# Roy-Kid/ADMP

Hardware: AMD Instinct MI355X
Metric: ns/day (electrostatics get_forces per 1 fs step, polarizable PME incl. SCF, moving atoms) (higher is better)
Workload: dtype f64; 1 GPU; water_pol_1024 (BASELINE configs[1]): 1024 polarizable MPID waters = 3072 atoms, seeded liquid box L=31.289 A, rc 4 A, f64; n_atoms=3072, n_pairs=42510, pair_list=fixed during the timed steps, parallelism=single GPU

## Files before the change

admp_amd/_lib.py:

```python
import ctypes

import numpy as np
import os

_HERE = os.path.dirname(os.path.abspath(__file__))
LIB_PATH = os.environ.get('ADMP_HIP_LIB') or os.path.join(_HERE, 'lib', 'libadmp_hip.so')

_c = ctypes
_vp, _i32, _i64, _dbl = _c.c_void_p, _c.c_int, _c.c_int64, _c.c_double
_u32, _u64 = _c.c_uint32, _c.c_uint64
_dp = _c.POINTER(_c.c_double)
_ip = _c.POINTER(_c.c_int)

PROTOTYPES = {
    'admp_version': (_c.c_char_p, []),
    'admp_create': (_i32, [_c.POINTER(_vp), _i32, _i32]),
    'admp_destroy': (_i32, [_vp]),
    'admp_last_error': (_c.c_char_p, [_vp]),
    'admp_set_stream': (_i32, [_vp, _vp]),
    'admp_use_default_stream': (_i32, [_vp]),
    'admp_synchronize': (_i32, [_vp]),
    'admp_set_topology': (_i32, [_vp, _i32, _vp, _vp, _vp, _vp, _vp]),
    'admp_set_ewald': (_i32, [_vp, _dbl, _i32, _i32, _i32, _i32, _i32]),
    'admp_set_pairs': (_i32, [_vp, _i64, _vp, _i32]),
# ... 28 lines not shown
    'admp_md_virial': (_i32, [_vp, _i32, _vp, _vp, _vp, _vp, _u64, _u64, _vp]),
    'admp_md_scale': (_i32, [_vp, _i32, _vp, _vp, _dbl]),
    'admp_md_mts_plan': (_i32, [_vp, _i32, _i32, _vp, _vp, _i32, _vp, _vp, _i32]),
    'admp_md_mts_step': (_i32, [_vp, _i32, _vp, _vp, _vp, _vp, _dp, _dbl, _dbl, _i32, _dbl, _dbl, _u64, _u64, _vp, _vp]),
    'admp_md_mts_info': (_i32, [_vp, _c.POINTER(_i64)]),
    'admp_md_con_plan': (_i32, [_vp, _i32, _i32, _vp, _vp, _i32]),
    'admp_md_con_step': (_i32, [_vp, _i32, _vp, _vp, _vp, _vp, _dp, _dbl, _dbl, _dbl, _dbl, _u64, _u64, _dbl, _i32, _vp]),
    'admp_md_con_kick': (_i32, [_vp, _i32, _vp, _vp, _vp, _vp, _dp, _dbl, _dbl, _dbl, _i32, _vp, _vp]),
    'admp_md_con_project': (_i32, [_vp, _i32, _vp, _vp, _vp, _dp, _dbl, _i32, _vp]),
    'admp_md_con_info': (_i32, [_vp, _c.POINTER(_i64)]),
    'admp_md_mol_plan': (_i32, [_vp, _i32, _vp, _i32]),
    'admp_md_mol_sums': (_i32, [_vp, _i32, _vp, _vp, _vp, _vp, _dp, _u64, _u64, _vp]),
    'admp_md_mol_scale': (_i32, [_vp, _i32, _vp, _vp, _vp, _dp, _dbl, _dbl]),
    'admp_md_mol_info': (_i32, [_vp, _c.POINTER(_i64)]),
    'admp_md_fire_step': (_i32, [_vp, _i32, _vp, _vp, _vp, _vp, _dp, _dbl, _u64, _vp]),
    'admp_neighbor_count': (_i32, [_vp, _i32, _vp, _dp, _dbl, _c.POINTER(_i64)]),
    'admp_neighbor_fill': (_i32, [_vp, _vp]),
    'admp_set_pairs_from_positions': (_i32, [_vp, _vp, _dp, _dbl]),
    'admp_slab_configure': (_i32, [_vp, _i32, _i32]),
    'admp_slab_info': (_i32, [_vp, _c.POINTER(_i64)]),
    'admp_scf_stats': (_i32, [_vp, _c.POINTER(_i64), _i32]),
    'admp_xpass_stats': (_i32, [_vp, _c.POINTER(_i64), _i32]),
    'admp_plane_mfma_stats': (_i32, [_vp, _c.POINTER(_i64), _i32]),
    'admp_mesh_convolve': (_i32, [_vp, _dp, _i32, _vp, _i32, _dp, _ip]),
    'admp_pair_real': (_i32, [_vp, _vp, _dp, _vp, _vp, _vp, _i32, _dp, _dp, _vp, _vp, _i32, _i32, _i32, _dp, _vp, _vp, _vp, _ip]),
    'admp_pair_rider_stats': (_i32, [_vp, _c.POINTER(_i64), _i32]),
    'admp_mesh_spread': (_i32, [_vp, _vp, _dp, _vp, _vp, _vp, _vp, _i32, _i32, _i32, _vp, _ip]),
    'admp_mesh_gather': (_i32, [_vp, _vp, _dp, _vp, _vp, _vp, _vp, _vp, _i32, _i32, _dp, _vp, _vp, _vp, _ip]),
    'admp_set_comm': (_i32, [_vp, _vp]),
    'admp_slab_home': (_i32, [_vp, _vp, _ip, _ip]),
    'admp_rccl_unique_id': (_i32, [_vp]),
    'admp_rccl_create': (_i32, [_c.POINTER(_vp), _i32, _vp, _i32, _i32]),
    'admp_rccl_destroy': (_i32, [_vp]),
    'admp_rccl_abort': (_i32, [_vp]),
    'admp_rccl_stats': (_i32, [_vp, _c.POINTER(_i64), _c.POINTER(_i64), _i32]),
    'admp_rccl_all_reduce': (_i32, [_vp, _vp, _i64, _i32, _i32, _vp]),
    'admp_rccl_all_to_all_v': (_i32, [_vp, _vp, _c.POINTER(_i64), _vp, _c.POINTER(_i64), _i32, _vp]),
    'admp_rccl_shift': (_i32, [_vp, _vp, _vp, _i64, _i32, _i32, _vp]),
    'admp_rccl_version': (_i32, [_ip]),
    'admp_rccl_last_error': (_c.c_char_p, []),
    'admp_set_comm_rccl': (_i32, [_vp, _vp]),
    'admp_profile_enable': (_i32, [_vp, _i32]),
    'admp_profile_filter': (_i32, [_vp, _c.c_char_p]),
    'admp_profile_reset': (_i32, [_vp]),
    'admp_profile_count': (_i32, [_vp]),
    'admp_profile_entry': (_i32, [_vp, _i32, _c.POINTER(_c.c_char_p), _dp, _c.POINTER(_i64)]),
# ... 59 lines not shown
```

admp_amd/csrc/dft_kernels.hip:

```cpp
#include "dft_lines.h"
#include "env.h"
#include "mfma.h"
#include "plane_mfma_plan.h"

namespace admp {

int dft_tile_cols(int N) { return dft_cols(N, dft_kq(), 0, 0); }
template <class T, int KQ, int JS>
__global__ __launch_bounds__(kDftBlock) void k_dft_z_r2c(int N, int nlines, int NL, int TK, const T* __restrict__ mesh,
                                                        Cx<T>* __restrict__ spec, const Cx<T>* __restrict__ twg,
                                                        long mesh_stride, long spec_stride) {
  mesh += blockIdx.y * mesh_stride;
  spec += blockIdx.y * spec_stride;
  const int H = (N - 1) / 2, Kh = N / 2 + 1;
  Cx<T>* tw = reinterpret_cast<Cx<T>*>(dft_smem);
  Cx<T>* p = tw + N;
  T* x0 = reinterpret_cast<T*>(p + H * NL);
  T* xn = x0 + NL;
  const int line0 = blockIdx.x * NL;
  const int nl = min(NL, nlines - line0);
  for (int t = threadIdx.x; t < N; t += kDftBlock) tw[t] = twg[t];
  for (int t = threadIdx.x; t < H * nl; t += kDftBlock) {
    const int l = t / H, jj = t - l * H;
    const T* x = mesh + (long)(line0 + l) * N;
// ... 422 lines not shown
        const int jb = wrap_add(ebase[2 * e], b, N2), bz = ebase[2 * e + 1];
#pragma unroll
        for (int c = 0; c < 6; ++c) {
          const T v = P0 * w[24 + c] + P1 * w[30 + c] + P2 * w[36 + c];
          const int jc = wrap_add(bz, c, N3);
          T* dst;
          if (jc == 0) dst = &x0[jb];
          else if (jc <= H3) dst = &p[(jc - 1) * N2 + jb].re;
          else if (2 * jc == N3) dst = &xn[jb];
          else dst = &p[(N3 - 1 - jc) * N2 + jb].im;
          atomicAdd(dst, v);
        }
      }
      __syncthreads();
    }
  }
  for (int t = threadIdx.x; t < H3 * N2; t += kZyBlock) {
    const Cx<T> ab = p[t];
    p[t] = Cx<T>{ab.re + ab.im, ab.re - ab.im};
  }
}

template <class T, int SIGN>
__device__ __forceinline__ void dft_y_unit(const PlaneMfmaPlan& mp, int u, const Cx<T>* Z, const Cx<T>* tw, Cx<T>* out, int os) {
  typedef typename Mfma<T>::Acc Acc;
  const int N = mp.N, H = mp.H, mt = u % mp.MT, ct = u / mp.MT;
  const int lane = threadIdx.x & 63, hi = plane_mfma_pos0(lane);
  const int i = plane_mfma_tw_row(mt, lane), c = plane_mfma_col(ct, lane), comp = plane_mfma_comp(lane);
  TwIdx ti(i < H ? i : 0, hi, N);
  const bool live = c < mp.ncols;
  const T* zc = reinterpret_cast<const T*>(Z + (live ? c : 0)) + comp;
  const int rs = 2 * mp.ncols;
  struct Ops { Cx<T> w; T b[2]; };
  auto fetch = [&](Ops& o, int kk) {
    o.w = tw[ti.m];
    ti.step();
    const bool ok = live && kk < H;
    o.b[0] = ok ? zc[(1 + kk) * rs] : T(0);
    o.b[1] = ok ? zc[(N - 1 - kk) * rs] : T(0);
  };
  Acc P = {0, 0, 0, 0}, R = {0, 0, 0, 0};
  T s0 = T(0);
  auto mul = [&](const Ops& o) {
    s0 += o.b[0];
    P = Mfma<T>::mma(o.w.re, o.b[0], P);
    R = Mfma<T>::mma(o.w.im, o.b[1], R);
  };
  Ops A, B;
  fetch(A, hi);
  for (int kk = hi; kk < mp.KP; kk += 8) {
    const bool two = kk + 4 < mp.KP;
    if (two) fetch(B, kk + 4);
    mul(A);
    if (kk + 8 < mp.KP) fetch(A, kk + 8);
    if (two) mul(B);
  }
  const T x0 = zc[0], xn = (N & 1) ? T(0) : zc[(N / 2) * rs];
  T* o = reinterpret_cast<T*>(out + (live ? c : 0)) + comp;
#pragma unroll
  for (int r = 0; r < 4; ++r) {
    const int k = plane_mfma_out_k(mt, lane, r);
    const T other = __shfl_xor(R[r], 8, 64);
    if (live && k <= H) {
      T base = x0 + P[r];
      if ((N & 1) == 0) base += (k & 1) ? -xn : xn;
      const T q = comp ? T(SIGN) * other : -T(SIGN) * other;
      o[2 * (long)k * os] = base + q;
      o[2 * (long)(N - k) * os] = base - q;
    }
  }
  if (mt == 0) {
    T s1 = (hi & 1) ? s0 : -s0;
    s0 += __shfl_xor(s0, 16, 64); s1 += __shfl_xor(s1, 16, 64);
    s0 += __shfl_xor(s0, 32, 64); s1 += __shfl_xor(s1, 32, 64);
    if (hi == 0 && live) {
      o[0] = x0 + s0 + xn;
      if ((N & 1) == 0) o[2 * (long)(N / 2) * os] = x0 + s1 + (((N / 2) & 1) ? -xn : xn);
    }
  }
}

template <class T>
__device__ __forceinline__ void dft_z_unit(const PlaneMfmaZPlan& zp, int u, const Cx<T>* p, const T* x0, const T* xn,
                                           const Cx<T>* tw, Cx<T>* Z) {
  typedef typename Mfma<T>::Acc Acc;
  const int N = zp.N, H = zp.H, mt = u % zp.MT, lt = u / zp.MT;
  const int lane = threadIdx.x & 63, hi = lane >> 4;
  const int kt = plane_mfma_z_tw_k(zp, mt, lane), l = plane_mfma_z_line(lt, lane);
  TwIdx ti((kt <= N / 2 ? kt : 0) - 1, hi, N);
  const bool live = l < zp.nlines;
  const Cx<T>* pl = p + (live ? l : 0);
  struct Ops { Cx<T> w, v; };
  auto fetch = [&](Ops& o, int kk) {
    o.w = tw[ti.m];
    ti.step();
    o.v = (live && kk < H) ? pl[kk * zp.nlines] : Cx<T>{T(0), T(0)};
  };
  Acc P = {0, 0, 0, 0}, R = {0, 0, 0, 0};
  auto mul = [&](const Ops& o) {
    P = Mfma<T>::mma(o.w.re, o.v.re, P);
    R = Mfma<T>::mma(o.w.im, o.v.im, R);
  };
// ... 108 lines not shown
    }
    ZY_TRACE_END(4);
    return;
  }
  for (int task = threadIdx.x; task < TK2 * Kl; task += kZyBlock) {
    const int g = task / Kl, c = task - g * Kl;
    int k[KQ];
#pragma unroll
    for (int q = 0; q < KQ; ++q) k[q] = (g + q * TK2 < Kh2) ? g + q * TK2 : 0;
    Cx<T> Xk[KQ], Xnk[KQ];
    dft_pair_outputs_rows<T, -1, KQ>(N2, k, Kl, Z + c, tw2, Xk, Xnk);
#pragma unroll
    for (int q = 0; q < KQ; ++q) {
      const int kq = g + q * TK2;
      if (kq < Kh2) {
        out[(long)kq * Kh + kz0 + c] = Xk[q];
        if (kq != 0 && 2 * kq != N2) out[(long)(N2 - kq) * Kh + kz0 + c] = Xnk[q];
      }
    }
  }
  ZY_TRACE_END(4);
}

template <class T, int KQ>
__global__ __launch_bounds__(kZyBlock) void k_dft_yz_inv(int N2, int N3, const Cx<T>* __restrict__ spec, T* __restrict__ mesh,
                                                         const Cx<T>* __restrict__ tw2g, const Cx<T>* __restrict__ tw3g,
                                                         long mesh_stride, long spec_stride, T* __restrict__ accum) {
  __shared__ int s_lines[2 * 160 + 2];
  __shared__ int s_nlines;
  const ZyLayout<T> L(N2, N3);
  const int Kh = N3 / 2 + 1, H2 = (N2 - 1) / 2;
  Cx<T>* tw3 = reinterpret_cast<Cx<T>*>(dft_smem + L.tw3);
  Cx<T>* tw2 = reinterpret_cast<Cx<T>*>(dft_smem + L.tw2);
  Cx<T>* V = reinterpret_cast<Cx<T>*>(dft_smem + L.a);
  Cx<T>* Z = reinterpret_cast<Cx<T>*>(dft_smem + L.b);
  const Cx<T>* in = spec + blockIdx.y * spec_stride + (long)blockIdx.x * N2 * Kh;
  T* plane = mesh + blockIdx.y * mesh_stride + (long)blockIdx.x * N2 * N3;
  T* acc = accum ? accum + (long)blockIdx.x * N2 * N3 : nullptr;
  const int Kh2 = N2 / 2 + 1, TK2 = (Kh2 + KQ - 1) / KQ;
  const int g0 = (int)(((long)TK2 * blockIdx.z) / gridDim.z), g1 = (int)(((long)TK2 * (blockIdx.z + 1)) / gridDim.z);
  ZY_TRACE(0);
  for (int t = threadIdx.x; t < N3; t += kZyBlock) tw3[t] = tw3g[t];
  for (int t = threadIdx.x; t < N2; t += kZyBlock) tw2[t] = tw2g[t];
  if (threadIdx.x == 0) {
    int n = 0;
    for (int g = g0; g < g1; ++g)
      for (int q = 0; q < KQ; ++q) {
        const int kq = g + q * TK2;
        if (kq >= Kh2) continue;
        s_lines[n++] = kq;
        if (kq != 0 && 2 * kq != N2) s_lines[n++] = N2 - kq;
      }
    s_nlines = n;
  }
  for (int t = threadIdx.x; t < (H2 + 1) * Kh; t += kZyBlock) {
    const int jj = t / Kh, c = t - jj * Kh;
    if (jj == H2) {
      Z[c] = in[c];
      if ((N2 & 1) == 0) Z[(N2 / 2) * Kh + c] = in[(long)(N2 / 2) * Kh + c];
      continue;
    }
    const Cx<T> a = in[(long)(1 + jj) * Kh + c], b = in[(long)(N2 - 1 - jj) * Kh + c];
    Z[(1 + jj) * Kh + c] = Cx<T>{a.re + b.re, a.im + b.im};
    Z[(N2 - 1 - jj) * Kh + c] = Cx<T>{a.re - b.re, a.im - b.im};
  }
  __syncthreads();
  ZY_TRACE(1);
  for (int task = threadIdx.x; task < (g1 - g0) * Kh; task += kZyBlock) {
    const int g = g0 + task / Kh, c = task % Kh;
    int k[KQ];
#pragma unroll
    for (int q = 0; q < KQ; ++q) k[q] = (g + q * TK2 < Kh2) ? g + q * TK2 : 0;
    Cx<T> Xk[KQ], Xnk[KQ];
    dft_pair_outputs_rows<T, +1, KQ>(N2, k, Kh, Z + c, tw2, Xk, Xnk);
#pragma unroll
    for (int q = 0; q < KQ; ++q) {
      const int kq = g + q * TK2;
      if (kq < Kh2) {
        V[kq * Kh + c] = Xk[q];
        if (kq != 0 && 2 * kq != N2) V[(N2 - kq) * Kh + c] = Xnk[q];
      }
    }
  }
  __syncthreads();
  ZY_TRACE(2);
  const int TK3 = (Kh + KQ - 1) / KQ, nl = s_nlines;
  for (int task = threadIdx.x; task < nl * TK3; task += kZyBlock) {
    const int l = s_lines[task / TK3], g = task % TK3;
    int j[KQ];
#pragma unroll
    for (int q = 0; q < KQ; ++q) j[q] = (g + q * TK3 < Kh) ? g + q * TK3 : 0;
    const Cx<T>* v = V + l * Kh;
    T xj[KQ], xnj[KQ];
    irdft_pair_outputs<T, KQ>(N3, j, 1, v + 1, v[0].re, (N3 & 1) ? T(0) : v[N3 / 2].re, tw3, xj, xnj);
    T* x = plane + (long)l * N3;
    T* ac = acc ? acc + (long)l * N3 : nullptr;
#pragma unroll
    for (int q = 0; q < KQ; ++q) {
      const int jq = g + q * TK3;
      if (jq < Kh) {
        x[jq] = xj[q];
        if (ac) ac[jq] += xj[q];
        if (jq != 0 && 2 * jq != N3) {
          x[N3 - jq] = xnj[q];
          if (ac) ac[N3 - jq] += xnj[q];
        }
      }
    }
  }
  ZY_TRACE_END(3);
// ... 64 lines not shown
  const size_t sh = dft_x_fixed_bytes(N, sizeof(T), false) + dft_x_col_bytes(N, sizeof(T), false) * (size_t)NC;
  const dim3 grid((Kh + NCt - 1) / NCt, K[1], 1);
#define XMIX(NTP)                                                                                                          \
  k_dft_x_mix<T, 2, 1, NTP><<<grid, kDftBlock, sh, st>>>(N, Kh, NC, TK, (long)K[1] * Kh, (long)Kh, K[2],                    \
                                                         reinterpret_cast<Cx<T>*>(spec), tabs, mix,                        \
                                                         reinterpret_cast<const Cx<T>*>(tw), energies, slot, spec_stride / 2)
  if (ntp == 1) XMIX(1); else if (ntp == 2) XMIX(2); else XMIX(4);
#undef XMIX
}
template <class T>
bool dft_zy_fits(const int K[3]) {
  static const bool off = !env_flag("ADMP_DFT_PLANES", true);
  return !off && 2 * K[0] <= 256 && ZyLayout<T>(K[1], K[2]).total + 2048 <= 160 * 1024;
}
template <class T>
bool dft_zy_spread_fits(const int K[3], int na) {
  static const int mx = env_int("ADMP_FUSE_SPREAD_MAX", 8192);
  return sizeof(T) == 8 && na > 0 && na <= mx && na <= kZySpreadMaxAtoms && dft_zy_fits<T>(K) && zy_spread_sub<T>(K[1], K[2]) >= 16;
}
template <class T>
bool launch_dft_zy(hipStream_t st, const int K[3], const T* tw, T* mesh, T* spec, int inverse, int nb, long mesh_stride,
                   long spec_stride, T* accum, const PlaneSpread<T>* sp, int* mfma_share) {
  const size_t sh = ZyLayout<T>(K[1], K[2]).total;
  const bool mf = sizeof(T) == 8 && !inverse && env_flag("ADMP_DFT_PLANE_MFMA", true) &&
                  (plane_mfma_y_plan(K[1], (K[2] / 2 + 1) / 2, kZyBlock / 64).CT > 0 ||
                   plane_mfma_z_plan(K[2], 0, (K[2] / 2 + 1) / 2, K[1], kZyBlock / 64).MT > 0);
  if (mfma_share) *mfma_share = mf ? 1 : 0;
  const Cx<T>* t1 = reinterpret_cast<const Cx<T>*>(tw) + K[0];
  const Cx<T>* t2 = t1 + K[1];
  const dim3 grid(K[0], nb, 2);
  static size_t attr_set[2] = {0, 0};
  if (inverse) {
    auto kern = k_dft_yz_inv<T, 2>;
    if (attr_set[1] < sh) { (void)hipFuncSetAttribute((const void*)kern, hipFuncAttributeMaxDynamicSharedMemorySize, (int)sh); attr_set[1] = sh; }
    kern<<<grid, kZyBlock, sh, st>>>(K[1], K[2], reinterpret_cast<const Cx<T>*>(spec), mesh, t1, t2, mesh_stride, spec_stride / 2,
                                     nb == 1 ? accum : nullptr);
    return accum != nullptr && nb == 1;
  }
  if constexpr (sizeof(T) == 8) {
    if (mf) {
      static size_t attr_mf[2] = {0, 0};
      auto kern = sp ? k_dft_zy_fwd<T, 2, true, true> : k_dft_zy_fwd<T, 2, false, true>;
      size_t& have = attr_mf[sp ? 1 : 0];
      if (have < sh) { (void)hipFuncSetAttribute((const void*)kern, hipFuncAttributeMaxDynamicSharedMemorySize, (int)sh); have = sh; }
      kern<<<grid, kZyBlock, sh, st>>>(K[1], K[2], mesh, reinterpret_cast<Cx<T>*>(spec), t1, t2, mesh_stride, spec_stride / 2,
                                       sp ? *sp : PlaneSpread<T>());
      return false;
    }
  }
  if (sp) {
    static size_t attr_sp = 0;
    auto kern = k_dft_zy_fwd<T, 2, true>;
    if (attr_sp < sh) { (void)hipFuncSetAttribute((const void*)kern, hipFuncAttributeMaxDynamicSharedMemorySize, (int)sh); attr_sp = sh; }
    kern<<<grid, kZyBlock, sh, st>>>(K[1], K[2], mesh, reinterpret_cast<Cx<T>*>(spec), t1, t2, mesh_stride, spec_stride / 2, *sp);
    return false;
// ... 24 lines not shown
```

admp_amd/csrc/engine.hip:

```cpp
#include <hip/hip_runtime.h>
#include <hip/hiprtc.h>
#include <rocfft/rocfft.h>

#include <algorithm>
#include <array>
#include <cmath>
#include <cstdio>
#include <cstring>
#include <map>
#include <memory>
#include <mutex>
#include <set>
#include <string>
#include <functional>
#include <vector>

#include "../../include/admp_hip.h"
#include "dev_buf.h"
#include "dft_math.h"
#include "disp_plan.h"
#include "handle.h"
#include "launch.h"
#include "rccl_comm.h"
#include "scf_policy.h"
// ... 22 lines not shown
  bool have_comm = false;
  admp_rccl* rccl = nullptr;
  void comm_fail(const char* what, int rc) {
    if (rccl) throw Err{ADMP_E_COMM, std::string(what) + ": " + rccl_error()};
    throw Err{ADMP_E_COMM, std::string("communicator callback ") + what + " returned " + std::to_string(rc)};
  }
  void c_all_reduce(void* buf, int64_t n, int dtype, int op, int tag) {
    const int rc = rccl ? rccl_all_reduce(rccl, stream, buf, n, dtype, op, tag) : comm.all_reduce(comm.ctx, buf, n, dtype, op, tag);
    if (rc != 0) comm_fail("all_reduce", rc);
  }
  void c_all_to_all_v(const void* send, const int64_t* sc, void* recv, const int64_t* rc_, int dtype, int tag) {
    const int rc = rccl ? rccl_all_to_all_v(rccl, stream, send, sc, recv, rc_, dtype, tag)
                        : comm.all_to_all_v(comm.ctx, send, sc, recv, rc_, dtype, tag);
    if (rc != 0) comm_fail("all_to_all_v", rc);
  }
  void c_shift(const void* send, void* recv, int64_t n, int dtype, int to_next, int tag) {
    const int rc = rccl ? rccl_shift(rccl, stream, send, recv, n, dtype, to_next, tag)
                        : comm.shift(comm.ctx, send, recv, n, dtype, to_next, tag);
    if (rc != 0) comm_fail("shift", rc);
  }
  int64_t scf_stats[8] = {0, 0, 0, 0, 0, 0, 0, 0};
  int64_t xpass_stats[2] = {0, 0};
  int64_t plane_mfma_stats[2] = {0, 0};
  int64_t pair_rider_stats[2] = {0, 0};
  const void* U_src = nullptr;
  const void* U_src_now = nullptr;
  double cutoff = 0.0;
  int ref_korder = 0;
  int keep_pol_sites = 0;
  int side_stream_on = 1;
  virtual void after_error() {}
  long nbr_gen = 0;
  NbrTable nbr_full;
  bool pruned = false;
  void unprune() {
    if (!pruned) return;
    nbr = nbr_full;
    nbr_full = NbrTable();
    pruned = false;
    ++nbr_gen;
  }
  EngineBase* nbr_src = nullptr;
  long nbr_src_gen = -1;
  static std::set<EngineBase*>& live() { static std::set<EngineBase*> s; return s; }
  static std::mutex& live_mu() { static std::mutex m; return m; }
  static bool is_live(EngineBase* e) { std::lock_guard<std::mutex> g(live_mu()); return live().count(e) != 0; }
// ... 763 lines not shown
        }
      });
      (void)accum;
      return false;
    }
    if (use_pfa) {
      const T* tw = pfa_tw.as<T>();
      { TIMED("dft_z_r2c"); launch_pfa_z<T>(stream, pfa, tw, mesh_p, spec_p, 0); }
      { TIMED("dft_y_fwd"); launch_pfa_y<T>(stream, pfa, tw, spec_p, 0); }
      DftTabs<T> tabs;
      tabs.p[0] = gtab;
      { TIMED("dft_x_kspace"); launch_pfa_x_conv<T>(stream, pfa, tw, spec_p, tabs, Ed, slot); }
      { TIMED("dft_y_inv"); launch_pfa_y<T>(stream, pfa, tw, spec_p, 1); }
      { TIMED("dft_z_c2r"); launch_pfa_z<T>(stream, pfa, tw, mesh_p, spec_p, 1); }
      return false;
    }
    if (use_dft) {
      const T* tw = dft_tw.as<T>();
      const bool planes = dft_zy_fits<T>(K);
      ARG_CHECK(!sp || planes, "internal: plane spread without the plane kernels");
      int mf = 0;
      if (planes && sp) { TIMED("dft_spread_zy_fwd"); launch_dft_zy<T>(stream, K, tw, mesh_p, spec_p, 0, 1, 0, 0, nullptr, sp, &mf); }
      else if (planes) { TIMED("dft_zy_fwd"); launch_dft_zy<T>(stream, K, tw, mesh_p, spec_p, 0, 1, 0, 0, nullptr, nullptr, &mf); }
      if (planes) ++plane_mfma_stats[mf ? 0 : 1];
      else {
        { TIMED("dft_z_r2c"); launch_dft_z<T>(stream, K, tw, mesh_p, spec_p, 0); }
        { TIMED("dft_y_fwd"); launch_dft_y<T>(stream, K, tw, spec_p, 0); }
      }
      DftTabs<T> tabs;
      tabs.p[0] = gtab;
      const T* ct = xctab_ok && gtab == gtabs[0].template as<T>() ? xctab.template as<T>() : nullptr;
      ++xpass_stats[ct ? 0 : 1];
      { TIMED("dft_x_kspace"); launch_dft_x_pass<T>(stream, K, tw, spec_p, tabs, Ed, slot, ct, rider, prider); }
      bool added;
      if (planes) {
        TIMED("dft_yz_inv");
        added = launch_dft_zy<T>(stream, K, tw, mesh_p, spec_p, 1, 1, 0, 0, accum, nullptr, &mf);
        ++plane_mfma_stats[mf ? 0 : 1];
      }
      else {
        { TIMED("dft_y_inv"); launch_dft_y<T>(stream, K, tw, spec_p, 1); }
        { TIMED("dft_z_c2r"); added = launch_dft_z<T>(stream, K, tw, mesh_p, spec_p, 1, 1, 0, 0, accum); }
      }
      return added;
    }
    if (use_fx) {
      run_plan("rocfft_r2c_yz", plan2_f, mesh_p, spec_p);
      { TIMED("fftx_kspace"); launch_fftx_conv<T>(stream, K, fx_tw.as<T>(), spec_p, gtab, Ed, slot, fx_khp); }
      run_plan("rocfft_c2r_yz", plan2_b, spec_p, mesh_o);
      return false;
    }
    fft_forward(mesh_p, spec_p);
    { TIMED("kspace"); launch_kspace<T>(stream, K, nyown(), gtab, spec_p, Ed, slot); }
    fft_inverse(spec_p, mesh_o);
    return false;
  }

  rocfft_plan plan2n_f[4] = {nullptr, nullptr, nullptr, nullptr}, plan2n_b[4] = {nullptr, nullptr, nullptr, nullptr};
  void ensure_batched_plans(int nb) {
    ARG_CHECK(nb >= 2 && nb <= 3 && use_fx && snranks == 1, "internal: batched y-z plans");
    if (plan2n_f[nb]) return;
// ... 2151 lines not shown
  return guarded(h, [&](EngineBase& e) {
    ARG_CHECK(rc >= 0.0, "negative cutoff");
    e.cutoff = rc;
  });
}
int admp_scf_stats(admp_handle* h, int64_t* out8, int reset) {
  return guarded(h, [&](EngineBase& e) {
    ARG_CHECK(out8, "null");
    for (int k = 0; k < 8; ++k) { out8[k] = e.scf_stats[k]; if (reset) e.scf_stats[k] = 0; }
  });
}
int admp_xpass_stats(admp_handle* h, int64_t* out2, int reset) {
  return guarded(h, [&](EngineBase& e) {
    ARG_CHECK(out2, "null");
    for (int k = 0; k < 2; ++k) { out2[k] = e.xpass_stats[k]; if (reset) e.xpass_stats[k] = 0; }
  });
}
int admp_plane_mfma_stats(admp_handle* h, int64_t* out2, int reset) {
  return guarded(h, [&](EngineBase& e) {
    ARG_CHECK(out2, "null");
    for (int k = 0; k < 2; ++k) { out2[k] = e.plane_mfma_stats[k]; if (reset) e.plane_mfma_stats[k] = 0; }
  });
}
int admp_mesh_convolve(admp_handle* h, const double* box, int which, void* mesh_inout, int on_device, double* E_out,
                       int32_t* info16) {
  return guarded(h, [&](EngineBase& e) { e.mesh_convolve(box, which, mesh_inout, on_device, E_out, info16); });
}
int admp_pair_real(admp_handle* h, const void* positions, const double* box, const void* Q_local, const void* pol,
                   const void* tholes, int n_scales, const double* mScales, const double* pScales, const void* U,
                   const void* F, int which, int flags, int on_device, double* E_out, void* grad, void* pot, void* fld,
                   int32_t* info4) {
  return guarded(h, [&](EngineBase& e) {
    e.pair_real(positions, box, Q_local, pol, tholes, n_scales, mScales, pScales, U, F, which, flags, on_device, E_out, grad,
                pot, fld, info4);
  });
}
int admp_mesh_spread(admp_handle* h, const void* positions, const double* box, const void* Q_local, const void* pol,
                     const void* tholes, const void* U, int which, int flags, int on_device, void* mesh_out, int32_t* info8) {
  return guarded(h, [&](EngineBase& e) {
    e.mesh_spread(positions, box, Q_local, pol, tholes, U, which, flags, on_device, mesh_out, info8);
  });
}
int admp_mesh_gather(admp_handle* h, const void* positions, const double* box, const void* Q_local, const void* pol,
                     const void* tholes, const void* U, const void* phi_in, int which, int on_device, double* E_out, void* pot,
                     void* grad, void* fld, int32_t* info4) {
  return guarded(h, [&](EngineBase& e) {
// ... 39 lines not shown
```

admp_amd/csrc/plane_mfma_plan.h:

```cpp
#pragma once
#include "dft_math.h"

namespace admp {

struct PlaneMfmaPlan {
  int N, H, KP;
  int ncols;
  int MT, CT;
  int nm;
  int nunits, Wm;
};
ADMP_HD PlaneMfmaPlan plane_mfma_y_plan(int N, int ncols, int nwaves) {
  PlaneMfmaPlan p;
  p.N = N; p.H = (N - 1) / 2; p.KP = (p.H + 3) & ~3;
  p.ncols = ncols;
  p.MT = (p.H + 15) / 16;
  p.CT = p.H < 16 ? 0 : (ncols + 7) / 8;
  p.nm = 8 * p.CT < ncols ? 8 * p.CT : ncols;
  p.nunits = p.MT * p.CT;
  p.Wm = p.nunits < nwaves ? p.nunits : nwaves;
  return p;
}
ADMP_HD int plane_mfma_tw_row(int mt, int lane) { return 16 * mt + (lane & 15); }
ADMP_HD int plane_mfma_col(int ct, int lane) { return 8 * ct + (lane & 7); }
// ... 59 lines not shown
ADMP_HD int plane_mfma_z_out_k(const PlaneMfmaZPlan& p, int mt, int lane, int r) { return p.k0 + 16 * mt + (lane >> 4) + 4 * r; }
ADMP_HD bool plane_mfma_z_operand_live(const PlaneMfmaZPlan& p, int kk, int l) { return kk < p.H && l < p.nlines; }

template <class T>
inline void plane_mfma_z_unit_host(const PlaneMfmaZPlan& p, int u, const Cx<T>* ps, const T* x0, const T* xn, const Cx<T>* tw,
                                   Cx<T>* X, T* sums) {
  const int N = p.N, mt = u % p.MT, lt = u / p.MT;
  for (int l = 16 * lt; l < 16 * lt + 16 && l < p.nlines; ++l)
    for (int k = p.k0 + 16 * mt; k < p.k0 + 16 * mt + 16 && k < p.k0 + p.nout; ++k) {
      T P = T(0), R = T(0);
      for (int kk = 0; kk < p.KP; ++kk) {
        const int m = (int)(((long)k * (1 + kk)) % N);
        const Cx<T> v = plane_mfma_z_operand_live(p, kk, l) ? ps[kk * p.nlines + l] : Cx<T>{T(0), T(0)};
        P += tw[m].re * v.re;
        R += tw[m].im * v.im;
      }
      T re = x0[l] + P;
      if ((N & 1) == 0) re += (k & 1) ? -xn[l] : xn[l];
      X[l * p.nout + k - p.k0] = Cx<T>{re, -R};
      if (sums) { sums[(size_t)(l * p.nout + k - p.k0) * 2] = P; sums[(size_t)(l * p.nout + k - p.k0) * 2 + 1] = R; }
    }
}

}
```

admp_amd/pme.py:

```python
import ctypes
import math
import warnings

import numpy as np
import torch

from . import _lib, settings
from ._device import HipForceBase

DIELECTRIC = 1389.35455846
DEFAULT_THOLE_WIDTH = 0.3


def setup_ewald_parameters(rc, ethresh, box):
    box = np.asarray(box.detach().cpu() if isinstance(box, torch.Tensor) else box, dtype=np.float64)
    kappa = math.sqrt(-math.log(2 * ethresh)) / rc
    K1 = math.ceil(2 * kappa * box[0, 0] / 3 / ethresh ** 0.2)
    K2 = math.ceil(2 * kappa * box[1, 1] / 3 / ethresh ** 0.2)
    K3 = math.ceil(2 * kappa * box[2, 2] / 3 / ethresh ** 0.2)
    if settings.FFT_FRIENDLY_MESH:
        K1, K2, K3 = (next_smooth(int(k)) for k in (K1, K2, K3))
    return kappa, int(K1), int(K2), int(K3)


# ... 334 lines not shown
                                      self._ptr(pol_t), self._ptr(th_t), len(mS), _lib.darr(mS), _lib.darr(pS), self._ptr(U),
                                      out)
        _lib.check(self._h, rc, 'admp_pscale_grad')
        return np.array(out[:], dtype=np.float64)

    def get_mscale_gradient(self, positions, box, pairs, Q_local, mScales):
        return self._mscale_gradient(0, positions, box, pairs, self._pad_Q(Q_local), 9, len(self._host64(mScales)))

    def scf_stats(self, reset=False):
        out = (ctypes.c_int64 * 8)()
        _lib.check(self._h, self._L.admp_scf_stats(self._h, out, 1 if reset else 0), 'admp_scf_stats')
        keys = ('plain', 'speculative', 'speculative_failed', 'chained', 'chained_too_short', 'chained_too_long',
                'wasted_increments', 'jacobi_steps')
        return dict(zip(keys, (int(v) for v in out)))

    def xpass_stats(self, reset=False):
        out = (ctypes.c_int64 * 2)()
        _lib.check(self._h, self._L.admp_xpass_stats(self._h, out, 1 if reset else 0), 'admp_xpass_stats')
        return {'circulant': int(out[0]), 'transforms': int(out[1])}

    def plane_mfma_stats(self, reset=False):
        out = (ctypes.c_int64 * 2)()
        _lib.check(self._h, self._L.admp_plane_mfma_stats(self._h, out, 1 if reset else 0), 'admp_plane_mfma_stats')
        return {'matrix_share': int(out[0]), 'vector': int(out[1])}

    def pair_rider_stats(self, reset=False):
        out = (ctypes.c_int64 * 2)()
        _lib.check(self._h, self._L.admp_pair_rider_stats(self._h, out, 1 if reset else 0), 'admp_pair_rider_stats')
        return {'rode': int(out[0]), 'own_launch': int(out[1])}

    def pair_real(self, positions, box, pairs, Q_local, mScales, pol=None, tholes=None, pScales=None, U=None, which=0,
                  flags=1, field=None):
        self._use_current_stream()
        L, h, na = self._L, self._h, self.n_atoms
        self.set_pairs(pairs)
        pos = self._real(positions, (na, 3))
        Q = self._pad_Q(Q_local)
        mS = self._host64(mScales)
        pol_t = th_t = U_t = pS = F_t = None
        if self.lpol:
            pol_t, th_t, U_t = self._real(pol, (na,)), self._real(tholes, (na,)), self._real(U, (na, 3))
            pS = _lib.darr(self._host64(pScales, len(mS)))
            F_t = self._real(field, (na, 3)) if field is not None else None

        def new(k):
            return torch.empty((na, k), dtype=self._dtype, device=self._device)
        grad, pot = (new(3), new(9)) if which == 0 else (None, None)
# ... 56 lines not shown
```

include/admp_hip.h:

```cpp
#ifndef ADMP_HIP_H
#define ADMP_HIP_H

#include <stdint.h>

#ifdef __cplusplus
extern "C" {
#endif

typedef struct admp_handle admp_handle;

enum {
  ADMP_OK = 0,
  ADMP_E_ARG = -1,
  ADMP_E_HIP = -2,
  ADMP_E_FFT = -3,
  ADMP_E_NOGPU = -4,
  ADMP_E_STATE = -5,
  ADMP_E_COMM = -6
};

const char* admp_version(void);

int admp_create(admp_handle** out, int device, int precision );
int admp_destroy(admp_handle* h);
// ... 129 lines not shown
} admp_comm;
int admp_slab_configure(admp_handle* h, int rank, int nranks);
int admp_set_comm(admp_handle* h, const admp_comm* comm);
int admp_slab_info(admp_handle* h, int64_t* out11);
typedef struct admp_rccl admp_rccl;
enum { ADMP_RCCL_ID_BYTES = 128, ADMP_RCCL_NTAGS = 8 };
int admp_rccl_unique_id(void* out128);
int admp_rccl_create(admp_rccl** out, int device, const void* id128, int rank, int nranks);
int admp_rccl_destroy(admp_rccl* c);
int admp_rccl_abort(admp_rccl* c);
int admp_rccl_stats(admp_rccl* c, int64_t* bytes_out, int64_t* calls_out, int reset);
int admp_rccl_all_reduce(admp_rccl* c, void* buf, int64_t count, int dtype , int op , void* hip_stream);
int admp_rccl_all_to_all_v(admp_rccl* c, const void* send, const int64_t* send_counts, void* recv, const int64_t* recv_counts,
                           int dtype, void* hip_stream);
int admp_rccl_shift(admp_rccl* c, const void* send, void* recv, int64_t count, int dtype, int to_next, void* hip_stream);
int admp_rccl_version(int* version);
const char* admp_rccl_last_error(void);
int admp_set_comm_rccl(admp_handle* h, admp_rccl* c);
int admp_slab_home(admp_handle* h, int32_t* home_out, int* n_home, int* n_import);

int admp_scf_stats(admp_handle* h, int64_t* out8, int reset);
int admp_xpass_stats(admp_handle* h, int64_t* out2, int reset);
int admp_plane_mfma_stats(admp_handle* h, int64_t* out2, int reset);
#define ADMP_MESH_INFO_WORDS 16
#define ADMP_MESH_PATH_ROCFFT 0
#define ADMP_MESH_PATH_FUSED_X 1
#define ADMP_MESH_PATH_DIRECT_LINES 2
#define ADMP_MESH_PATH_DIRECT_PLANES 3
#define ADMP_MESH_PATH_TWO_LEVEL 4
int admp_mesh_convolve(admp_handle* h, const double* box, int which, void* mesh_inout, int on_device, double* E_out,
                       int32_t* info16);
int admp_pair_real(admp_handle* h, const void* positions, const double* box, const void* Q_local, const void* pol,
                   const void* tholes, int n_scales, const double* mScales, const double* pScales, const void* U,
                   const void* F, int which, int flags, int on_device, double* E_out, void* grad, void* pot, void* fld,
                   int32_t* info4);
#define ADMP_SPREAD_FORM_SCAN 0
#define ADMP_SPREAD_FORM_PLANES 1
#define ADMP_SPREAD_FORM_BRICKS 2
#define ADMP_SPREAD_FORM_PLANE_KERNEL 3
int admp_mesh_spread(admp_handle* h, const void* positions, const double* box, const void* Q_local, const void* pol,
                     const void* tholes, const void* U, int which, int flags, int on_device, void* mesh_out, int32_t* info8);
int admp_mesh_gather(admp_handle* h, const void* positions, const double* box, const void* Q_local, const void* pol,
                     const void* tholes, const void* U, const void* phi_in, int which, int on_device, double* E_out, void* pot,
                     void* grad, void* fld, int32_t* info4);
int admp_pair_rider_stats(admp_handle* h, int64_t* out2, int reset);

// ... 11 lines not shown
```

Baseline: 526.5 ns/day.

## Use MFMA matrix units for inverse y/z plane DFT in PME

Extends the MFMA-based plane DFT path, previously forward-only, to the inverse y and z transforms. The y and z DFT work within each block is split into 16-row wave units and run through f64 MFMA accumulations, replacing the scalar per-thread loops. It adds a line-split plan and new stats counters, and it can be turned off with ADMP_DFT_PLANE_MFMA_INV. Risks are extra kernel complexity and register pressure, plus possible differences in summation order.

```diff
diff --git a/admp_amd/_lib.py b/admp_amd/_lib.py
--- a/admp_amd/_lib.py
+++ b/admp_amd/_lib.py
@@ -74,6 +74,7 @@
     'admp_scf_stats': (_i32, [_vp, _c.POINTER(_i64), _i32]),
     'admp_xpass_stats': (_i32, [_vp, _c.POINTER(_i64), _i32]),
     'admp_plane_mfma_stats': (_i32, [_vp, _c.POINTER(_i64), _i32]),
+    'admp_plane_mfma_stats4': (_i32, [_vp, _c.POINTER(_i64), _i32]),
     'admp_mesh_convolve': (_i32, [_vp, _dp, _i32, _vp, _i32, _dp, _ip]),
     'admp_pair_real': (_i32, [_vp, _vp, _dp, _vp, _vp, _vp, _i32, _dp, _dp, _vp, _vp, _i32, _i32, _i32, _dp, _vp, _vp, _vp, _ip]),
     'admp_pair_rider_stats': (_i32, [_vp, _c.POINTER(_i64), _i32]),
diff --git a/admp_amd/csrc/dft_kernels.hip b/admp_amd/csrc/dft_kernels.hip
--- a/admp_amd/csrc/dft_kernels.hip
+++ b/admp_amd/csrc/dft_kernels.hip
@@ -468,15 +468,15 @@
 }
 
 template <class T, int SIGN>
-__device__ __forceinline__ void dft_y_unit(const PlaneMfmaPlan& mp, int u, const Cx<T>* Z, const Cx<T>* tw, Cx<T>* out, int os) {
+__device__ __forceinline__ void dft_y_unit_rows(int N, int H, int KP, int ncols, int ib, int kl, int ct, bool w0, bool wn,
+                                                const Cx<T>* Z, const Cx<T>* tw, Cx<T>* out, int os) {
   typedef typename Mfma<T>::Acc Acc;
-  const int N = mp.N, H = mp.H, mt = u % mp.MT, ct = u / mp.MT;
   const int lane = threadIdx.x & 63, hi = plane_mfma_pos0(lane);
-  const int i = plane_mfma_tw_row(mt, lane), c = plane_mfma_col(ct, lane), comp = plane_mfma_comp(lane);
-  TwIdx ti(i < H ? i : 0, hi, N);
-  const bool live = c < mp.ncols;
+  const int i = ib + (lane & 15), c = plane_mfma_col(ct, lane), comp = plane_mfma_comp(lane);
+  TwIdx ti(i < kl ? i : 0, hi, N);
+  const bool live = c < ncols;
   const T* zc = reinterpret_cast<const T*>(Z + (live ? c : 0)) + comp;
-  const int rs = 2 * mp.ncols;
+  const int rs = 2 * ncols;
   struct Ops { Cx<T> w; T b[2]; };
   auto fetch = [&](Ops& o, int kk) {
     o.w = tw[ti.m];
@@ -494,20 +494,20 @@
   };
   Ops A, B;
   fetch(A, hi);
-  for (int kk = hi; kk < mp.KP; kk += 8) {
-    const bool two = kk + 4 < mp.KP;
+  for (int kk = hi; kk < KP; kk += 8) {
+    const bool two = kk + 4 < KP;
     if (two) fetch(B, kk + 4);
     mul(A);
-    if (kk + 8 < mp.KP) fetch(A, kk + 8);
+    if (kk + 8 < KP) fetch(A, kk + 8);
     if (two) mul(B);
   }
   const T x0 = zc[0], xn = (N & 1) ? T(0) : zc[(N / 2) * rs];
   T* o = reinterpret_cast<T*>(out + (live ? c : 0)) + comp;
 #pragma unroll
   for (int r = 0; r < 4; ++r) {
-    const int k = plane_mfma_out_k(mt, lane, r);
+    const int k = 1 + ib + (lane >> 4) + 4 * r;
     const T other = __shfl_xor(R[r], 8, 64);
-    if (live && k <= H) {
+    if (live && k <= kl) {
       T base = x0 + P[r];
       if ((N & 1) == 0) base += (k & 1) ? -xn : xn;
       const T q = comp ? T(SIGN) * other : -T(SIGN) * other;
@@ -515,15 +515,27 @@
       o[2 * (long)(N - k) * os] = base - q;
     }
   }
-  if (mt == 0) {
+  if (w0 || wn) {
     T s1 = (hi & 1) ? s0 : -s0;
     s0 += __shfl_xor(s0, 16, 64); s1 += __shfl_xor(s1, 16, 64);
     s0 += __shfl_xor(s0, 32, 64); s1 += __shfl_xor(s1, 32, 64);
     if (hi == 0 && live) {
-      o[0] = x0 + s0 + xn;
-      if ((N & 1) == 0) o[2 * (long)(N / 2) * os] = x0 + s1 + (((N / 2) & 1) ? -xn : xn);
-    }
-  }
+      if (w0) o[0] = x0 + s0 + xn;
+      if (wn && (N & 1) == 0) o[2 * (long)(N / 2) * os] = x0 + s1 + (((N / 2) & 1) ? -xn : xn);
+    }
+  }
+}
+
+template <class T, int SIGN>
+__device__ __forceinline__ void dft_y_unit(const PlaneMfmaPlan& mp, int u, const Cx<T>* Z, const Cx<T>* tw, Cx<T>* out, int os) {
+  const int mt = u % mp.MT, ct = u / mp.MT;
+  dft_y_unit_rows<T, SIGN>(mp.N, mp.H, mp.KP, mp.ncols, plane_mfma_tw_row(mt, 0), mp.H, ct, mt == 0, mt == 0, Z, tw, out, os);
+}
+template <class T>
+__device__ __forceinline__ void dft_y_unit_inv(const PlaneMfmaInvYPlan& yp, int u, const Cx<T>* Z, const Cx<T>* tw, Cx<T>* V) {
+  const int mt = u % yp.MT, ct = u / yp.MT;
+  dft_y_unit_rows<T, +1>(yp.N, yp.H, yp.KP, yp.ncols, plane_mfma_inv_y_kb(yp, mt) - 1, plane_mfma_inv_y_ke(yp, mt) - 1, ct,
+                         mt == 0 && yp.s.own0, mt == 0 && yp.s.ownn, Z, tw, V, yp.ncols);
 }
 
 template <class T>
@@ -678,7 +690,71 @@
   ZY_TRACE_END(4);
 }
 
-template <class T, int KQ>
+template <class T>
+__device__ __forceinline__ void dft_z_unit_inv(const PlaneMfmaInvZPlan& zp, int u, const Cx<T>* V, int Kh, const int* lines,
+                                               const Cx<T>* tw, T* plane, T* acc) {
+  typedef typename Mfma<T>::Acc Acc;
+  const int N = zp.N, H = zp.H, jt = u % zp.JT, lt = u / zp.JT;
+  const int lane = threadIdx.x & 63, hi = lane >> 4;
+  const int li = plane_mfma_inv_z_op_line(lt, lane), j = plane_mfma_inv_z_tw_j(jt, lane);
+  TwIdx ti((j <= H ? j : 1) - 1, hi, N);
+  const bool live = li < zp.nlines;
+  const Cx<T>* v = V + (live ? lines[li] : 0) * Kh;
+  struct Ops { Cx<T> w, a; };
+  auto fetch = [&](Ops& o, int kk) {
+    o.w = tw[ti.m];
+    ti.step();
+    o.a = (live && kk < H) ? v[1 + kk] : Cx<T>{T(0), T(0)};
+  };
+  Acc P = {0, 0, 0, 0}, R = {0, 0, 0, 0};
+  T s0 = T(0);
+  auto mul = [&](const Ops& o) {
+    s0 += o.a.re;
+    P = Mfma<T>::mma(o.a.re, o.w.re, P);
+    R = Mfma<T>::mma(o.a.im, o.w.im, R);
+  };
+  Ops A, B;
+  fetch(A, hi);
+  for (int kk = hi; kk < zp.KP; kk += 8) {
+    const bool two = kk + 4 < zp.KP;
+    if (two) fetch(B, kk + 4);
+    mul(A);
+    if (kk + 8 < zp.KP) fetch(A, kk + 8);
+    if (two) mul(B);
+  }
+#pragma unroll
+  for (int r = 0; r < 4; ++r) {
+    const int lo = plane_mfma_inv_z_out_line(lt, lane, r);
+    if (lo < zp.nlines && j <= H) {
+      const int l = lines[lo];
+      T base = V[l * Kh].re + T(2) * P[r];
+      if ((N & 1) == 0) { const T Xn = V[l * Kh + N / 2].re; base += (j & 1) ? -Xn : Xn; }
+      const T a = base - T(2) * R[r], b = base + T(2) * R[r];
+      plane[(long)l * N + j] = a;
+      plane[(long)l * N + N - j] = b;
+      if (acc) { acc[(long)l * N + j] += a; acc[(long)l * N + N - j] += b; }
+    }
+  }
+  if (jt == 0) {
+    T s1 = (hi & 1) ? s0 : -s0;
+    s0 += __shfl_xor(s0, 16, 64); s1 += __shfl_xor(s1, 16, 64);
+    s0 += __shfl_xor(s0, 32, 64); s1 += __shfl_xor(s1, 32, 64);
+    if (hi == 0 && live) {
+      const long o = (long)lines[li] * N;
+      const T X0 = v[0].re, Xn = (N & 1) ? T(0) : v[N / 2].re;
+      const T a = X0 + T(2) * s0 + Xn;
+      plane[o] = a;
+      if (acc) acc[o] += a;
+      if ((N & 1) == 0) {
+        const T b = X0 + T(2) * s1 + (((N / 2) & 1) ? -Xn : Xn);
+        plane[o + N / 2] = b;
+        if (acc) acc[o + N / 2] += b;
+      }
+    }
+  }
+}
+
+template <class T, int KQ, bool MF = false>
 __global__ __launch_bounds__(kZyBlock) void k_dft_yz_inv(int N2, int N3, const Cx<T>* __restrict__ spec, T* __restrict__ mesh,
                                                          const Cx<T>* __restrict__ tw2g, const Cx<T>* __restrict__ tw3g,
                                                          long mesh_stride, long spec_stride, T* __restrict__ accum) {
@@ -698,7 +774,11 @@
   ZY_TRACE(0);
   for (int t = threadIdx.x; t < N3; t += kZyBlock) tw3[t] = tw3g[t];
   for (int t = threadIdx.x; t < N2; t += kZyBlock) tw2[t] = tw2g[t];
-  if (threadIdx.x == 0) {
+  if constexpr (MF) {
+    const PlaneInvSplit sl = plane_inv_split(N2, (int)blockIdx.z, (int)gridDim.z);
+    for (int t = threadIdx.x; t < sl.nlines; t += kZyBlock) s_lines[t] = plane_inv_line(sl, t);
+    if (threadIdx.x == 0) s_nlines = sl.nlines;
+  } else if (threadIdx.x == 0) {
     int n = 0;
     for (int g = g0; g < g1; ++g)
       for (int q = 0; q < KQ; ++q) {
@@ -722,7 +802,13 @@
   }
   __syncthreads();
   ZY_TRACE(1);
-  for (int task = threadIdx.x; task < (g1 - g0) * Kh; task += kZyBlock) {
+  bool yshare = false;
+  if constexpr (MF) {
+    const PlaneMfmaInvYPlan yp = plane_mfma_inv_y_plan(N2, Kh, (int)blockIdx.z, (int)gridDim.z, kZyBlock / 64);
+    yshare = yp.nunits > 0;
+    for (int u = threadIdx.x >> 6; u < yp.nunits; u += yp.Wm) dft_y_unit_inv<T>(yp, u, Z, tw2, V);
+  }
+  for (int task = yshare ? (g1 - g0) * Kh : (int)threadIdx.x; task < (g1 - g0) * Kh; task += kZyBlock) {
     const int g = g0 + task / Kh, c = task % Kh;
     int k[KQ];
 #pragma unroll
@@ -741,7 +827,13 @@
   __syncthreads();
   ZY_TRACE(2);
   const int TK3 = (Kh + KQ - 1) / KQ, nl = s_nlines;
-  for (int task = threadIdx.x; task < nl * TK3; task += kZyBlock) {
+  bool zshare = false;
+  if constexpr (MF) {
+    const PlaneMfmaInvZPlan zp = plane_mfma_inv_z_plan(N3, nl, kZyBlock / 64);
+    zshare = zp.nunits > 0;
+    for (int u = threadIdx.x >> 6; u < zp.nunits; u += zp.Wm) dft_z_unit_inv<T>(zp, u, V, Kh, s_lines, tw3, plane, acc);
+  }
+  for (int task = zshare ? nl * TK3 : (int)threadIdx.x; task < nl * TK3; task += kZyBlock) {
     const int l = s_lines[task / TK3], g = task % TK3;
     int j[KQ];
 #pragma unroll
@@ -852,15 +944,30 @@
 bool launch_dft_zy(hipStream_t st, const int K[3], const T* tw, T* mesh, T* spec, int inverse, int nb, long mesh_stride,
                    long spec_stride, T* accum, const PlaneSpread<T>* sp, int* mfma_share) {
   const size_t sh = ZyLayout<T>(K[1], K[2]).total;
-  const bool mf = sizeof(T) == 8 && !inverse && env_flag("ADMP_DFT_PLANE_MFMA", true) &&
-                  (plane_mfma_y_plan(K[1], (K[2] / 2 + 1) / 2, kZyBlock / 64).CT > 0 ||
-                   plane_mfma_z_plan(K[2], 0, (K[2] / 2 + 1) / 2, K[1], kZyBlock / 64).MT > 0);
+  bool mf = sizeof(T) == 8 && env_flag("ADMP_DFT_PLANE_MFMA", true);
+  if (mf && inverse)
+    mf = env_flag("ADMP_DFT_PLANE_MFMA_INV", true) &&
+         (plane_mfma_inv_y_plan(K[1], K[2] / 2 + 1, 0, 2, kZyBlock / 64).nunits > 0 ||
+          plane_mfma_inv_z_plan(K[2], plane_inv_split(K[1], 0, 2).nlines, kZyBlock / 64).nunits > 0);
+  else if (mf)
+    mf = plane_mfma_y_plan(K[1], (K[2] / 2 + 1) / 2, kZyBlock / 64).CT > 0 ||
+         plane_mfma_z_plan(K[2], 0, (K[2] / 2 + 1) / 2, K[1], kZyBlock / 64).MT > 0;
   if (mfma_share) *mfma_share = mf ? 1 : 0;
   const Cx<T>* t1 = reinterpret_cast<const Cx<T>*>(tw) + K[0];
   const Cx<T>* t2 = t1 + K[1];
   const dim3 grid(K[0], nb, 2);
   static size_t attr_set[2] = {0, 0};
   if (inverse) {
+    if constexpr (sizeof(T) == 8) {
+      if (mf) {
+        static size_t attr_inv_mf = 0;
+        auto kern = k_dft_yz_inv<T, 2, true>;
+        if (attr_inv_mf < sh) { (void)hipFuncSetAttribute((const void*)kern, hipFuncAttributeMaxDynamicSharedMemorySize, (int)sh); attr_inv_mf = sh; }
+        kern<<<grid, kZyBlock, sh, st>>>(K[1], K[2], reinterpret_cast<const Cx<T>*>(spec), mesh, t1, t2, mesh_stride, spec_stride / 2,
+                                         nb == 1 ? accum : nullptr);
+        return accum != nullptr && nb == 1;
+      }
+    }
     auto kern = k_dft_yz_inv<T, 2>;
     if (attr_set[1] < sh) { (void)hipFuncSetAttribute((const void*)kern, hipFuncAttributeMaxDynamicSharedMemorySize, (int)sh); attr_set[1] = sh; }
     kern<<<grid, kZyBlock, sh, st>>>(K[1], K[2], reinterpret_cast<const Cx<T>*>(spec), mesh, t1, t2, mesh_stride, spec_stride / 2,
diff --git a/admp_amd/csrc/engine.hip b/admp_amd/csrc/engine.hip
--- a/admp_amd/csrc/engine.hip
+++ b/admp_amd/csrc/engine.hip
@@ -68,6 +68,7 @@
   int64_t scf_stats[8] = {0, 0, 0, 0, 0, 0, 0, 0};
   int64_t xpass_stats[2] = {0, 0};
   int64_t plane_mfma_stats[2] = {0, 0};
+  int64_t plane_mfma_stats4[4] = {0, 0, 0, 0};
   int64_t pair_rider_stats[2] = {0, 0};
   const void* U_src = nullptr;
   const void* U_src_now = nullptr;
@@ -877,7 +878,7 @@
       int mf = 0;
       if (planes && sp) { TIMED("dft_spread_zy_fwd"); launch_dft_zy<T>(stream, K, tw, mesh_p, spec_p, 0, 1, 0, 0, nullptr, sp, &mf); }
       else if (planes) { TIMED("dft_zy_fwd"); launch_dft_zy<T>(stream, K, tw, mesh_p, spec_p, 0, 1, 0, 0, nullptr, nullptr, &mf); }
-      if (planes) ++plane_mfma_stats[mf ? 0 : 1];
+      if (planes) { ++plane_mfma_stats[mf ? 0 : 1]; ++plane_mfma_stats4[mf ? 0 : 1]; }
       else {
         { TIMED("dft_z_r2c"); launch_dft_z<T>(stream, K, tw, mesh_p, spec_p, 0); }
         { TIMED("dft_y_fwd"); launch_dft_y<T>(stream, K, tw, spec_p, 0); }
@@ -891,7 +892,8 @@
       if (planes) {
         TIMED("dft_yz_inv");
         added = launch_dft_zy<T>(stream, K, tw, mesh_p, spec_p, 1, 1, 0, 0, accum, nullptr, &mf);
-        ++plane_mfma_stats[mf ? 0 : 1];
+        ++plane_mfma_stats[1];
+        ++plane_mfma_stats4[mf ? 2 : 3];
       }
       else {
         { TIMED("dft_y_inv"); launch_dft_y<T>(stream, K, tw, spec_p, 1); }
@@ -3089,6 +3091,12 @@
     for (int k = 0; k < 2; ++k) { out2[k] = e.plane_mfma_stats[k]; if (reset) e.plane_mfma_stats[k] = 0; }
   });
 }
+int admp_plane_mfma_stats4(admp_handle* h, int64_t* out4, int reset) {
+  return guarded(h, [&](EngineBase& e) {
+    ARG_CHECK(out4, "null");
+    for (int k = 0; k < 4; ++k) { out4[k] = e.plane_mfma_stats4[k]; if (reset) e.plane_mfma_stats4[k] = 0; }
+  });
+}
 int admp_mesh_convolve(admp_handle* h, const double* box, int which, void* mesh_inout, int on_device, double* E_out,
                        int32_t* info16) {
   return guarded(h, [&](EngineBase& e) { e.mesh_convolve(box, which, mesh_inout, on_device, E_out, info16); });
diff --git a/admp_amd/csrc/plane_mfma_plan.h b/admp_amd/csrc/plane_mfma_plan.h
--- a/admp_amd/csrc/plane_mfma_plan.h
+++ b/admp_amd/csrc/plane_mfma_plan.h
@@ -105,4 +105,152 @@
     }
 }
 
-}
+struct PlaneInvSplit {
+  int N, Kh2, TK, g0, g1;
+  int kb[2], kn[2];
+  int own0, ownn;
+  int nlines;
+};
+ADMP_HD PlaneInvSplit plane_inv_split(int N, int z, int nz) {
+  PlaneInvSplit s;
+  const int H = (N - 1) / 2;
+  s.N = N; s.Kh2 = N / 2 + 1; s.TK = (s.Kh2 + 1) / 2;
+  s.g0 = (int)(((long)s.TK * z) / nz); s.g1 = (int)(((long)s.TK * (z + 1)) / nz);
+  for (int r = 0; r < 2; ++r) {
+    int b = s.g0 + r * s.TK, e = s.g1 + r * s.TK;
+    if (b < 1) b = 1;
+    if (e > H + 1) e = H + 1;
+    s.kb[r] = b; s.kn[r] = e > b ? e - b : 0;
+  }
+  s.own0 = s.g0 == 0 && s.g1 > 0;
+  const int gn = N / 2 - s.TK;
+  s.ownn = (N & 1) == 0 && ((N / 2 >= s.g0 && N / 2 < s.g1) || (gn >= s.g0 && gn < s.g1));
+  s.nlines = 2 * (s.kn[0] + s.kn[1]) + s.own0 + s.ownn;
+  return s;
+}
+ADMP_HD int plane_inv_line(const PlaneInvSplit& s, int idx) {
+  if (idx < s.kn[0]) return s.kb[0] + idx;
+  idx -= s.kn[0];
+  if (idx < s.kn[1]) return s.kb[1] + idx;
+  idx -= s.kn[1];
+  if (idx < s.kn[0]) return s.N - (s.kb[0] + idx);
+  idx -= s.kn[0];
+  if (idx < s.kn[1]) return s.N - (s.kb[1] + idx);
+  idx -= s.kn[1];
+  if (idx == 0 && s.own0) return 0;
+  return s.N / 2;
+}
+
+struct PlaneMfmaInvYPlan {
+  int N, H, KP, ncols;
+  PlaneInvSplit s;
+  int T[2], MT, CT;
+  int nunits, Wm;
+};
+ADMP_HD PlaneMfmaInvYPlan plane_mfma_inv_y_plan(int N, int ncols, int z, int nz, int nwaves) {
+  PlaneMfmaInvYPlan p;
+  p.N = N; p.H = (N - 1) / 2; p.KP = (p.H + 3) & ~3;
+  p.ncols = ncols;
+  p.s = plane_inv_split(N, z, nz);
+  const bool share = p.H >= 16;
+  p.T[0] = share ? (p.s.kn[0] + 15) / 16 : 0;
+  p.T[1] = share ? (p.s.kn[1] + 15) / 16 : 0;
+  p.MT = p.T[0] + p.T[1];
+  p.CT = p.MT > 0 ? (ncols + 7) / 8 : 0;
+  p.nunits = p.MT * p.CT;
+  p.Wm = p.nunits < nwaves ? p.nunits : nwaves;
+  return p;
+}
+ADMP_HD int plane_mfma_inv_y_kb(const PlaneMfmaInvYPlan& p, int mt) {
+  return mt < p.T[0] ? p.s.kb[0] + 16 * mt : p.s.kb[1] + 16 * (mt - p.T[0]);
+}
+ADMP_HD int plane_mfma_inv_y_ke(const PlaneMfmaInvYPlan& p, int mt) {
+  const int r = mt < p.T[0] ? 0 : 1, e = p.s.kb[r] + p.s.kn[r], t = plane_mfma_inv_y_kb(p, mt) + 16;
+  return t < e ? t : e;
+}
+ADMP_HD bool plane_mfma_inv_y_operand_live(const PlaneMfmaInvYPlan& p, int kk, int c) { return kk < p.H && c < p.ncols; }
+template <class T>
+inline void plane_mfma_inv_y_unit_host(const PlaneMfmaInvYPlan& p, int u, const Cx<T>* Z, const Cx<T>* tw, Cx<T>* X, T* sums) {
+  const int N = p.N, H = p.H, mt = u % p.MT, ct = u / p.MT;
+  const int kb = plane_mfma_inv_y_kb(p, mt), ke = plane_mfma_inv_y_ke(p, mt);
+  for (int c = 8 * ct; c < 8 * ct + 8 && c < p.ncols; ++c) {
+    const Cx<T> x0 = Z[c], xn = (N & 1) ? Cx<T>{T(0), T(0)} : Z[(N / 2) * p.ncols + c];
+    for (int k = kb; k < ke; ++k) {
+      T P[2] = {T(0), T(0)}, R[2] = {T(0), T(0)};
+      for (int kk = 0; kk < p.KP; ++kk) {
+        const bool live = plane_mfma_inv_y_operand_live(p, kk, c);
+        const int m = (int)(((long)k * (1 + kk)) % N);
+        const Cx<T> a = live ? Z[(1 + kk) * p.ncols + c] : Cx<T>{T(0), T(0)};
+        const Cx<T> b = live ? Z[(N - 1 - kk) * p.ncols + c] : Cx<T>{T(0), T(0)};
+        P[0] += tw[m].re * a.re; P[1] += tw[m].re * a.im;
+        R[0] += tw[m].im * b.re; R[1] += tw[m].im * b.im;
+      }
+      T bre = x0.re + P[0], bim = x0.im + P[1];
+      if ((N & 1) == 0) { bre += (k & 1) ? -xn.re : xn.re; bim += (k & 1) ? -xn.im : xn.im; }
+      X[k * p.ncols + c] = Cx<T>{bre - R[1], bim + R[0]};
+      X[(N - k) * p.ncols + c] = Cx<T>{bre + R[1], bim - R[0]};
+      if (sums) { T* s = sums + (size_t)(k * p.ncols + c) * 4; s[0] = P[0]; s[1] = P[1]; s[2] = R[0]; s[3] = R[1]; }
+    }
+    if (mt == 0 && (p.s.own0 || p.s.ownn)) {
+      T s[4][2] = {{T(0), T(0)}, {T(0), T(0)}, {T(0), T(0)}, {T(0), T(0)}};
+      for (int kk = 0; kk < H; ++kk) { s[kk & 3][0] += Z[(1 + kk) * p.ncols + c].re; s[kk & 3][1] += Z[(1 + kk) * p.ncols + c].im; }
+      if (p.s.own0)
+        X[c] = Cx<T>{x0.re + ((s[0][0] + s[1][0]) + (s[2][0] + s[3][0])) + xn.re, x0.im + ((s[0][1] + s[1][1]) + (s[2][1] + s[3][1])) + xn.im};
+      if (p.s.ownn) {
+        const T sg = ((N / 2) & 1) ? T(-1) : T(1);
+        X[(N / 2) * p.ncols + c] = Cx<T>{x0.re + ((s[1][0] - s[0][0]) + (s[3][0] - s[2][0])) + sg * xn.re,
+                                         x0.im + ((s[1][1] - s[0][1]) + (s[3][1] - s[2][1])) + sg * xn.im};
+      }
+    }
+  }
+}
+
+struct PlaneMfmaInvZPlan {
+  int N, H, KP, nlines;
+  int JT, LT;
+  int nunits, Wm;
+};
+ADMP_HD PlaneMfmaInvZPlan plane_mfma_inv_z_plan(int N, int nlines, int nwaves) {
+  PlaneMfmaInvZPlan p;
+  p.N = N; p.H = (N - 1) / 2; p.KP = (p.H + 3) & ~3;
+  p.nlines = nlines;
+  p.JT = p.H < 16 ? 0 : (p.H + 15) / 16;
+  p.LT = (nlines + 15) / 16;
+  p.nunits = p.JT * p.LT;
+  p.Wm = p.nunits < nwaves ? p.nunits : nwaves;
+  return p;
+}
+ADMP_HD int plane_mfma_inv_z_op_line(int lt, int lane) { return 16 * lt + (lane & 15); }
+ADMP_HD int plane_mfma_inv_z_tw_j(int jt, int lane) { return 1 + 16 * jt + (lane & 15); }
+ADMP_HD int plane_mfma_inv_z_out_line(int lt, int lane, int r) { return 16 * lt + (lane >> 4) + 4 * r; }
+ADMP_HD bool plane_mfma_inv_z_operand_live(const PlaneMfmaInvZPlan& p, int kk, int li) { return kk < p.H && li < p.nlines; }
+template <class T>
+inline void plane_mfma_inv_z_unit_host(const PlaneMfmaInvZPlan& p, int u, const Cx<T>* V, const Cx<T>* tw, T* x, T* sums) {
+  const int N = p.N, H = p.H, Kh = N / 2 + 1, jt = u % p.JT, lt = u / p.JT;
+  for (int li = 16 * lt; li < 16 * lt + 16 && li < p.nlines; ++li) {
+    const Cx<T>* v = V + (size_t)li * Kh;
+    const T X0 = v[0].re, Xn = (N & 1) ? T(0) : v[N / 2].re;
+    for (int j = 1 + 16 * jt; j < 17 + 16 * jt && j <= H; ++j) {
+      T P = T(0), R = T(0);
+      for (int kk = 0; kk < p.KP; ++kk) {
+        const int m = (int)(((long)j * (1 + kk)) % N);
+        const Cx<T> a = plane_mfma_inv_z_operand_live(p, kk, li) ? v[1 + kk] : Cx<T>{T(0), T(0)};
+        P += a.re * tw[m].re;
+        R += a.im * tw[m].im;
+      }
+      T base = X0 + T(2) * P;
+      if ((N & 1) == 0) base += (j & 1) ? -Xn : Xn;
+      x[(size_t)li * N + j] = base - T(2) * R;
+      x[(size_t)li * N + N - j] = base + T(2) * R;
+      if (sums) { sums[((size_t)li * (H + 1) + j) * 2] = P; sums[((size_t)li * (H + 1) + j) * 2 + 1] = R; }
+    }
+    if (jt == 0) {
+      T s[4] = {T(0), T(0), T(0), T(0)};
+      for (int kk = 0; kk < H; ++kk) s[kk & 3] += v[1 + kk].re;
+      x[(size_t)li * N] = X0 + T(2) * ((s[0] + s[1]) + (s[2] + s[3])) + Xn;
+      if ((N & 1) == 0) x[(size_t)li * N + N / 2] = X0 + T(2) * ((s[1] - s[0]) + (s[3] - s[2])) + (((N / 2) & 1) ? -Xn : Xn);
+    }
+  }
+}
+
+}
diff --git a/admp_amd/pme.py b/admp_amd/pme.py
--- a/admp_amd/pme.py
+++ b/admp_amd/pme.py
@@ -380,7 +380,9 @@
     def plane_mfma_stats(self, reset=False):
         out = (ctypes.c_int64 * 2)()
         _lib.check(self._h, self._L.admp_plane_mfma_stats(self._h, out, 1 if reset else 0), 'admp_plane_mfma_stats')
-        return {'matrix_share': int(out[0]), 'vector': int(out[1])}
+        out4 = (ctypes.c_int64 * 4)()
+        _lib.check(self._h, self._L.admp_plane_mfma_stats4(self._h, out4, 1 if reset else 0), 'admp_plane_mfma_stats4')
+        return {'matrix_share': int(out[0]), 'vector': int(out[1]), 'inverse_share': int(out4[2]), 'inverse_vector': int(out4[3])}
 
     def pair_rider_stats(self, reset=False):
         out = (ctypes.c_int64 * 2)()
diff --git a/include/admp_hip.h b/include/admp_hip.h
--- a/include/admp_hip.h
+++ b/include/admp_hip.h
@@ -175,6 +175,7 @@
 int admp_scf_stats(admp_handle* h, int64_t* out8, int reset);
 int admp_xpass_stats(admp_handle* h, int64_t* out2, int reset);
 int admp_plane_mfma_stats(admp_handle* h, int64_t* out2, int reset);
+int admp_plane_mfma_stats4(admp_handle* h, int64_t* out4, int reset);
 #define ADMP_MESH_INFO_WORDS 16
 #define ADMP_MESH_PATH_ROCFFT 0
 #define ADMP_MESH_PATH_FUSED_X 1
```

Result: faster. 543.6 ns/day (median of 6 runs) (+3.3%).
